# lachinov/brats2019

Hardware: AMD Instinct MI355X
Metric: volumes_per_sec_fwd_bwd_128cubed_x4ch (higher is better)
Workload: dtype bf16

## Files before the change

### brats2019_amd/_lib.py

```python
from __future__ import annotations

import ctypes as C
import os

import torch

_PKG = os.path.dirname(os.path.abspath(__file__))
LIB_PATH = os.environ.get("RU_LIB_PATH") or os.path.join(_PKG, "lib", "libresunet_hip.so")

_lib = None
PRECISIONS = {"f32": 0, "bf16x3": 1}
GRAD_PRECISIONS = {"bf16x3": 1, "bf16": 2}
FUSE_GN_BWD_STATS, FUSE_GN_BWD_APPLY, FUSE_SIDE_STREAM, FUSE_BATCH_WREDUCE, FUSE_TAIL_FINALIZE, FUSE_PW_DGRAD = 1, 2, 4, 8, 16, 32

_vp, _f, _d, _i, _sz = C.c_void_p, C.c_float, C.c_double, C.c_int, C.c_size_t

SIGNATURES = {
    "ru_last_error": (C.c_char_p, []),
    "ru_version": (_i, []),
    "ru_device_ok": (_i, []),
    "ru_conv3d_workspace_bytes": (_sz, [_i] * 7),
    "ru_conv3d_fwd": (_i, [_vp, _vp, _vp, _vp] + [_i] * 7 + [_vp, _sz, _vp]),
    "ru_conv3d_bwd_data": (_i, [_vp, _vp, _vp] + [_i] * 7 + [_vp, _sz, _vp]),
    "ru_conv3d_fwd_p": (_i, [_vp, _vp, _vp, _vp] + [_i] * 8 + [_vp, _sz, _vp]),
# ... 86 lines not shown
    "ru_case_stats": (_i, [_vp, _vp, _i, _i, _i, _i, C.POINTER(_i), C.POINTER(_i), _vp, _sz, _vp]),
    "ru_case_prepare": (_i, [_vp, _vp, _vp, _i, _i, _i, _i, C.POINTER(_i), C.POINTER(_i), C.POINTER(_i), C.POINTER(_i), _i, C.c_uint, _vp]),
    "ru_tta_merge_box": (_i, [_vp, _i, C.c_uint, _vp, _vp, _vp, _i, _i, _i, _i, C.POINTER(_i), C.POINTER(_i), _vp]),
    "ru_cc_workspace_bytes": (_sz, [_i, _i, _i]),
    "ru_cc_reject": (_i, [_vp, _i, _i, _i, _d, _vp, _sz, _vp]),
    "ru_paste_labels": (_i, [_vp, _vp, _i, _i, _i, C.POINTER(_i), C.POINTER(_i), _vp]),
    "ru_postprocess_workspace_bytes": (_sz, [_i, _i, _i, _i]),
    "ru_postprocess_regions": (_i, [_vp, _vp, _i, _i, _i, _i, C.POINTER(C.c_longlong), C.POINTER(C.c_ulonglong), C.c_uint, C.c_uint, _i, _vp, _vp, _vp, _vp, _sz, _vp]),
    "ru_ens_accumulate": (_i, [_vp, _i, C.c_uint, _vp, _i, _i, _i, _i, _i, C.POINTER(_i), C.POINTER(_i), _vp]),
    "ru_ens_finalize": (_i, [_vp, _i, _vp, _vp, _vp, _i, _sz, _vp]),
    "ru_ens_accumulate_finalize": (_i, [_vp, _i, C.c_uint, _vp, _i, _i, _vp, _vp, _vp, _i, _i, _i, _i, C.POINTER(_i), C.POINTER(_i), _vp]),
    "ru_ens_argmax": (_i, [_vp, _i, _vp, _i, _sz, _vp]),
    "ru_paste_probs": (_i, [_vp, _vp, _i, _i, _i, _i, C.POINTER(_i), C.POINTER(_i), _vp]),
    "ru_unc_accumulate": (_i, [_vp, _i, C.c_uint, _vp, _vp, _i, _i, _i, _i, _i, C.POINTER(_i), C.POINTER(_i), _vp]),
    "ru_unc_accumulate_finalize": (_i, [_vp, _i, C.c_uint, _vp, _vp, _i, _i, _i, _vp, _vp, _vp, _vp, _i, _i, _i, _i, C.POINTER(_i), C.POINTER(_i), _vp]),
    "ru_unc_finalize": (_i, [_vp, _vp, _i, _i, _i, _vp, _vp, _vp, _vp, _i, _sz, _vp]),
    "ru_unc_histogram": (_i, [_vp, _vp, _vp, _i, _i, _i, _vp, _vp, _vp]),
    "ru_unc_score": (_i, [_vp, C.POINTER(_i), _i, _vp, _vp, _vp]),
    "ru_paste_u8c": (_i, [_vp, _vp, _i, _i, _i, _i, C.POINTER(_i), C.POINTER(_i), _vp]),
    "ru_zscore_workspace_bytes": (_sz, [_i, _sz]),
    "ru_zscore_stats": (_i, [_vp, _vp, _i, _sz, _vp, _sz, _vp]),
    "ru_augment_patch": (_i, [_vp, _vp, _vp, _vp, _i, _i, _i, _i, _vp, _vp, _vp, _i, _vp, _vp, _vp, _vp, _vp]),
    "ru_augment_patch_soft": (_i, [_vp, _vp, _vp, _vp, _vp, _i, _i, _i, _i, _vp, _vp, _vp, _i, _vp, _vp, _vp, _vp, _vp]),
    "ru_augment_patch_affine": (_i, [_vp, _vp, _vp, _vp, _vp, _i, _i, _i, _i, _vp, _vp, _vp, _i, _vp, _vp, _i, _vp, _vp, _vp]),
    "ru_elastic_workspace_bytes": (_sz, [_i, _i, _i]),
    "ru_elastic_noise": (_i, [C.c_ulonglong, _i, _i, _i, _vp, _vp]),
    "ru_elastic_field": (_i, [_vp, _d, _d, _i, _i, _i, _vp, _vp, _sz, _vp]),
    "ru_elastic_warp": (_i, [_vp, _i, _vp, _i, _vp, _i, _i, _i, _i, _vp, _vp, _vp, _vp, _vp]),
    "ru_intensity_workspace_bytes": (_sz, [_i, _i, _i, _i]),
    "ru_intensity_augment": (_i, [_vp, _vp, _i, _i, _i, _i, _vp, _vp, _sz, _vp]),
    "ru_layout_convert": (_i, [_vp, _vp, _i, _i, _sz, _i, _vp]),
    "ru_upsample2x_trilinear_fwd_l": (_i, [_vp, _vp] + [_i] * 5 + [_f, _vp]),
    "ru_upsample2x_trilinear_bwd_l": (_i, [_vp, _vp] + [_i] * 5 + [_vp]),
    "ru_conv3d_fwd_l": (_i, [_vp, _vp, _vp, _vp] + [_i] * 7 + [_vp, _sz, _vp]),
    "ru_conv3d_bwd_weight_l": (_i, [_vp, _vp, _vp] + [_i] * 7 + [_vp, _sz, _vp]),
    "ru_conv1_l_workspace_bytes": (_sz, [_i, _i, _i]),
    "ru_conv1_l": (_i, [_vp, _i, _vp, _i, _vp, _i, _vp, _vp, _i, _vp, _f, _vp, _f, _i, _i, _sz, _i, _i, _i, _i, _vp, _vp, _f, _vp, _sz,
                        C.POINTER(_i), C.POINTER(_i), _vp, _sz, _vp]),
    "ru_conv3_l_workspace_bytes": (_sz, [_i] * 7),
    "ru_conv3_l": (_i, [_vp, _vp, _vp, _vp] + [_i] * 8 + [_vp, _vp, _vp, _f, _vp, _vp, _i, _i, _vp, _vp, _f, _vp, _sz, C.POINTER(_i), C.POINTER(_i), _vp, _sz, _vp]),
    "ru_wgrad1_l_workspace_bytes": (_sz, [_i, _i, _i, _sz]),
    "ru_wgrad3_l_workspace_bytes": (_sz, [_i] * 7),
    "ru_wgrad3_l": (_i, [_vp, _vp, _vp] + [_i] * 8 + [_vp, _vp, _f, _i, _i, _vp, _vp, _vp, _vp, _vp, _f, _vp, C.POINTER(_i), _vp, _sz, _vp]),
    "ru_wgrad1_l": (_i, [_vp, _vp, _i, _vp, _vp, _i, _i, _i, _i, _sz] + [_i] * 6 + [_vp, _i, _vp, _vp, _f, C.POINTER(_i), _vp, _sz, _vp]),
}


CRIT_KINDS = {"Dice_loss_joint": 0, "BCE_Loss": 1, "MSE_Loss": 2, "CE_Loss": 3, "Dice1D": 4, "GDL_joint": 5, "sens_loss_joint": 6,
              "Dice_loss_separate": 7}
CRIT_MOMENTS, CRIT_MAX_TERMS = 7, 8
CRIT_MASK_LOGS, CRIT_MASK_ALL = (1 << 4) | (1 << 5), 0x7F
CRIT_M_D2 = 6

CONF_PROB, CONF_LABEL, OVERLAP_MAX_LABELS = 0, 1, 8
OVERLAP_MODES = {"itk": 0, "wt": 1, "validate": 2}

UNC_MEASURES = {"std": 0, "entropy": 1}
UNC_REGIONS, UNC_LEVELS, UNC_CLASSES = 3, 101, 4

SURFACE_PROB, SURFACE_LABEL, SURFACE_REGIONS, SURFACE_COUNTS = 0, 1, 3, 6
SURFACE_COLUMNS = {"dice": 0, "sensitivity": 1, "specificity": 2, "hd95": 3}

LESION_COUNTS, LESION_TABLE_COLUMNS, LESION_CHUNK = 6, 5, 8
LESION_COLUMNS = {"dice": 0, "hd95": 1}

POSTPROCESS_MASKS, POSTPROCESS_LABELS, POSTPROCESS_REGIONS, POSTPROCESS_STATS = 0, 1, 3, 6
# ... 77 lines not shown
```

### brats2019_amd/csrc/engine.hip

```cpp
#include "ru_common.h"

#include <vector>
#include <math.h>
#include <stdlib.h>
#include <string.h>

#include <string>
#include <vector>

namespace ru {

static thread_local char g_err[512] = "";
void set_error(const char* fmt, ...) {
    va_list ap;
    va_start(ap, fmt);
    vsnprintf(g_err, sizeof(g_err), fmt, ap);
    va_end(ap);
}
int hip_fail(hipError_t e, const char* what) {
    set_error("%s: %s", what, hipGetErrorString(e));
    return RU_EHIP;
}

constexpr float kSlope = 1e-2f;
// ... 1554 lines not shown

extern "C" int ru_tta_merge(const float* probs, int K, unsigned flips, float* mean_out, unsigned char* mask, unsigned long long* counts,
                            int C, int D, int H, int W, ru_stream_t stream) {
    RU_REQUIRE(probs && mask && counts, "ru_tta_merge: null argument");
    return tta_merge_launch(probs, K, flips, mean_out, mask, counts, C, D, H, W, (hipStream_t)stream);
}
extern "C" int ru_compose_labels(const unsigned char* mask, const unsigned long long* counts, unsigned long long et_min, unsigned char* labels,
                                 size_t V, ru_stream_t stream) {
    RU_REQUIRE(mask && counts && labels, "ru_compose_labels: null argument");
    return compose_labels_launch(mask, counts, et_min, labels, V, (hipStream_t)stream);
}

extern "C" int ru_dice_accumulate(const unsigned long long* counts, double* acc, int N, int C, int nacc, ru_stream_t stream) {
    return dice_accumulate_launch(counts, acc, N, C, nacc, (hipStream_t)stream);
}
extern "C" int ru_dice_counts(const float* p, const float* g, unsigned long long* counts, int N, int C, size_t V, ru_stream_t stream) {
    RU_REQUIRE(p && g && counts && N > 0 && C > 0, "ru_dice_counts: bad argument");
    return dice_counts_launch(p, g, counts, N * C, V, (hipStream_t)stream);
}

extern "C" int ru_layout_convert(const float* src, float* dst, int N, int C, size_t V, int to_c16, ru_stream_t stream) {
    RU_REQUIRE(src && dst && N > 0, "ru_layout_convert: bad argument");
    return layout_convert_launch(src, dst, N, C, V, to_c16, (hipStream_t)stream);
}

extern "C" int ru_upsample2x_trilinear_fwd_l(const float* x, float* y, int N, int C, int D, int H, int W, float out_slope, ru_stream_t stream) {
    RU_REQUIRE(x && y && N > 0 && C > 0 && D > 0 && H > 0 && W > 0, "ru_upsample2x_trilinear_fwd_l: bad argument");
    return up2_fwd16_launch(x, y, N, C, D, H, W, out_slope, (hipStream_t)stream);
}
extern "C" int ru_upsample2x_trilinear_bwd_l(const float* dy, float* dx, int N, int C, int D, int H, int W, ru_stream_t stream) {
    RU_REQUIRE(dy && dx && N > 0 && C > 0 && D > 0 && H > 0 && W > 0, "ru_upsample2x_trilinear_bwd_l: bad argument");
    return up2_bwd16_launch(dy, dx, N, C, D, H, W, (hipStream_t)stream);
}
extern "C" int ru_conv3d_fwd_l(const float* x, const float* w, const float* bias, float* y, int N, int Cin, int Cout, int D, int H, int W,
                               int flags, void* ws, size_t ws_bytes, ru_stream_t stream) {
    RU_REQUIRE(x && w && y, "ru_conv3d_fwd_l: null argument");
    const Switches sw = switches_from_env();
    hipStream_t s = (hipStream_t)stream;
    WsCarver C(ws, ws_bytes);
    Conv3Args a{};
    void* wf = C.take(conv3_sb_frag_bytes(Cin, Cout) / 4 + 64);
    RU_WS_OK(C);
    const bool f32 = (flags & 16) != 0;
    a.products = (flags & 32) ? 2 : 0;
    RU_REQUIRE(!f32 || ((flags & 3) != 0 && !(flags & (4 | 8))), "ru_conv3d_fwd_l: the exact-f32 form needs a voxel-major side and takes neither the 4-channel copy nor a split-form input");
    const bool gop = (flags & 64) && !f32 && (flags & 3) == 3 && !(flags & (4 | 8)) && !bias && conv3_mxg_usable(sw, N, Cin, Cout, D, H, W);
    int rc = f32 ? conv3_f32c_pack_weights(w, wf, Cin, Cout, 0, s) : conv3_sb_pack_weights(w, wf, Cin, Cout, 0, s, gop);
    if (rc) return rc;
    a.mode = f32 ? RU_PREC_F32 : RU_PREC_BF16X3; a.wfrag = wf;
    a.in_c16 = flags & 1; a.out_c16 = (flags >> 1) & 1;
    a.in_s16 = (flags >> 3) & 1;
    RU_REQUIRE(!a.in_s16 || a.in_c16, "ru_conv3d_fwd_l: the split form is a voxel-major layout");
    a.x = x; a.bias = bias; a.y = y; a.N = N; a.Cin = Cin; a.Cout = Cout; a.D = D; a.H = H; a.W = W;
    if (gop) {
        const size_t nvox = (size_t)N * D * H * W;
        float* g16 = C.take(nvox * 16);
        RU_WS_OK(C);
        rc = conv3_mxg_split_launch(x, g16, nvox, s);
        if (rc) return rc;
        a.x = g16; a.in_s16 = 1; a.in_g16 = 1; a.products = 0;
    }
    if (flags & 4) {
        RU_REQUIRE(!(flags & 1) && conv3_sb4_usable(N, Cin, Cout, D, H, W), "ru_conv3d_fwd_l: shape does not fit the 4-channel kernel");
        const size_t V = (size_t)D * H * W;
        float* x4 = C.take((size_t)N * 4 * V);
        void* wf4 = C.take(conv3_sb4_frag_bytes(Cout) / 4 + 64);
// ... 209 lines not shown
```

### brats2019_amd/csrc/pointwise_c16.hip

```cpp
#include "pw_helpers.hpp"
#include "fin_tail.hpp"
#include <type_traits>
#include <stdlib.h>

namespace ru {

typedef float f32x4_c16 __attribute__((ext_vector_type(4)));
template <int I, int N, class F> __device__ __forceinline__ void static_for_c1_impl(F&& f) {
    if constexpr (I < N) { f(std::integral_constant<int, I>{}); static_for_c1_impl<I + 1, N>(f); }
}
template <int N, class F> __device__ __forceinline__ void static_for_c1(F&& f) { static_for_c1_impl<0, N>(f); }

static inline dim3 c16_grid(size_t V, int blocks_nc, unsigned cap = 2048) {
    size_t bx = (V * 4 + 255) / 256;
    if (bx > cap) bx = cap;
    if (bx < 1) bx = 1;
    return dim3((unsigned)bx, (unsigned)blocks_nc);
}

template <int RES, bool NT = false>
__global__ __launch_bounds__(256) void gn_apply16_kernel(const float* __restrict__ x, const float* __restrict__ scale, const float* __restrict__ shift,
                                                         const float* __restrict__ res, float* __restrict__ y, int C, size_t V, float slope,
                                                         const float* __restrict__ rscale, const float* __restrict__ rshift, float rslope) {
    const int nb = blockIdx.y, CB = C >> 4;
// ... 79 lines not shown
        }
    }
#pragma unroll
    for (int k = 0; k < 4; ++k) {
#pragma unroll
        for (int o = 4; o < 64; o <<= 1) { s1[k] += __shfl_xor(s1[k], o); s2[k] += __shfl_xor(s2[k], o); }
    }
    if (lane < 4) {
#pragma unroll
        for (int k = 0; k < 4; ++k) { red[wave][lane * 4 + k][0] = s1[k]; red[wave][lane * 4 + k][1] = s2[k]; }
    }
    __syncthreads();
    if (threadIdx.x < 16) {
        const int c = threadIdx.x;
        float* p = partials + (((size_t)n * C + cb * 16 + c) * nblk + blockIdx.x) * 2;
        stat_publish(p, (red[0][c][0] + red[1][c][0]) + (red[2][c][0] + red[3][c][0]), (red[0][c][1] + red[1][c][1]) + (red[2][c][1] + red[3][c][1]));
    }
    fin_tail(fin, partials, red_dyn + 128);
}
int gn_bwd_reduce16_launch(const float* x, const float* dy, const float* scale, const float* shift, const float* mean, const float* rstd,
                           float slope, float* partials, int N, int C, size_t V, int G, hipStream_t s, const FinTail* fin) {
    RU_REQUIRE(C % 16 == 0 && C % G == 0, "gn_bwd_reduce16: bad channel count");
    const int nblk = gn_bwd_tiles16(V);
    FinTail f{};
    if (fin) f = *fin;
    RU_REQUIRE(!f.ticket || (f.kind == 2 && f.nblk == nblk && f.N == N && f.C == C && f.G == G), "gn_bwd_reduce16: tail descriptor does not match the launch");
    const size_t lds = 512 + fin_tail_lds_bytes(f);
    RU_REQUIRE(lds <= 64 * 1024, "gn_bwd_reduce16: batch x channels too large for the in-launch finalize");
    hipLaunchKernelGGL(gn_bwd_reduce16_kernel, dim3(nblk, N * (C / 16)), dim3(256), lds, s, x, dy, scale, shift, mean, rstd, slope, partials, C, V, G, nblk, gn16_chunk(V), f);
    RU_CHECK_LAUNCH("gn_bwd_reduce16_kernel");
    return RU_OK;
}

__global__ __launch_bounds__(256) void gn_bwd_apply16_kernel(const float* __restrict__ x, const float* __restrict__ dy, const float* __restrict__ scale,
                                                             const float* __restrict__ shift, const float* __restrict__ coef, float slope,
                                                             float* __restrict__ dx, int C, size_t V) {
    const int nb = blockIdx.y, CB = C >> 4;
    const int n = nb / CB, cb = nb - n * CB;
    const int q = threadIdx.x & 3;
    const size_t row = (size_t)n * C + cb * 16 + 4 * q;
    float a[4], b[4], cA[4], cB[4], cC[4];
#pragma unroll
    for (int k = 0; k < 4; ++k) {
        a[k] = scale[row + k]; b[k] = shift[row + k];
        cA[k] = coef[(row + k) * 3]; cB[k] = coef[(row + k) * 3 + 1]; cC[k] = coef[(row + k) * 3 + 2];
    }
    const size_t base = (size_t)nb * V * 4, F = V * 4;
    const float4* xp = reinterpret_cast<const float4*>(x) + base;
    const float4* dp = reinterpret_cast<const float4*>(dy) + base;
    float4* op = reinterpret_cast<float4*>(dx) + base;
    for (size_t f = (size_t)blockIdx.x * 256 + threadIdx.x; f < F; f += (size_t)gridDim.x * 256) {
        const float4 t = xp[f], d = dp[f];
        float4 o;
        o.x = cA[0] * ((t.x * a[0] + b[0]) > 0.f ? d.x : d.x * slope) + (cB[0] * t.x + cC[0]);
        o.y = cA[1] * ((t.y * a[1] + b[1]) > 0.f ? d.y : d.y * slope) + (cB[1] * t.y + cC[1]);
        o.z = cA[2] * ((t.z * a[2] + b[2]) > 0.f ? d.z : d.z * slope) + (cB[2] * t.z + cC[2]);
        o.w = cA[3] * ((t.w * a[3] + b[3]) > 0.f ? d.w : d.w * slope) + (cB[3] * t.w + cC[3]);
        op[f] = o;
    }
}
__global__ __launch_bounds__(256) void gn_bwd_apply16_split_kernel(const float* __restrict__ x, const float* __restrict__ dy, const float* __restrict__ scale,
                                                                   const float* __restrict__ shift, const float* __restrict__ coef, float slope,
                                                                   float* __restrict__ dx, int C, size_t V) {
    const int nb = blockIdx.y, CB = C >> 4;
    const int n = nb / CB, cb = nb - n * CB;
    const int hf = threadIdx.x & 1;
    const size_t row = (size_t)n * C + cb * 16 + 8 * hf;
    float a[8], b[8], cA[8], cB[8], cC[8];
#pragma unroll
    for (int k = 0; k < 8; ++k) {
        a[k] = scale[row + k]; b[k] = shift[row + k];
        cA[k] = coef[(row + k) * 3]; cB[k] = coef[(row + k) * 3 + 1]; cC[k] = coef[(row + k) * 3 + 2];
    }
    const size_t base = (size_t)nb * V * 4, F = V * 2;
    const float4* xp = reinterpret_cast<const float4*>(x) + base;
    const float4* dp = reinterpret_cast<const float4*>(dy) + base;
    pw_u32x4* op = reinterpret_cast<pw_u32x4*>(dx) + base;
    for (size_t f = (size_t)blockIdx.x * 256 + threadIdx.x; f < F; f += (size_t)gridDim.x * 256) {
        const size_t v = f >> 1;
        const float4 t0 = xp[v * 4 + 2 * hf], t1 = xp[v * 4 + 2 * hf + 1], d0 = dp[v * 4 + 2 * hf], d1 = dp[v * 4 + 2 * hf + 1];
        const float tx[8] = {t0.x, t0.y, t0.z, t0.w, t1.x, t1.y, t1.z, t1.w}, dd[8] = {d0.x, d0.y, d0.z, d0.w, d1.x, d1.y, d1.z, d1.w};
        float o[8];
#pragma unroll
        for (int k = 0; k < 8; ++k) o[k] = cA[k] * ((tx[k] * a[k] + b[k]) > 0.f ? dd[k] : dd[k] * slope) + (cB[k] * tx[k] + cC[k]);
        pw_u32x4 hi, lo;
        pw_split8(o, hi, lo);
        op[v * 4 + hf] = hi;
        op[v * 4 + 2 + hf] = lo;
    }
}
int gn_bwd_apply16_launch(const float* x, const float* dy, const float* scale, const float* shift, const float* coef, float slope, float* dx,
                          int N, int C, size_t V, int split, hipStream_t s) {
    RU_REQUIRE(C % 16 == 0, "gn_bwd_apply16: C must be a multiple of 16");
    if (split) {
        size_t bx = (V * 2 + 255) / 256;
        if (bx > 2048) bx = 2048;
        hipLaunchKernelGGL(gn_bwd_apply16_split_kernel, dim3((unsigned)bx, (unsigned)(N * (C / 16))), dim3(256), 0, s, x, dy, scale, shift, coef, slope, dx, C, V);
    } else {
        hipLaunchKernelGGL(gn_bwd_apply16_kernel, c16_grid(V, N * (C / 16)), dim3(256), 0, s, x, dy, scale, shift, coef, slope, dx, C, V);
    }
    RU_CHECK_LAUNCH("gn_bwd_apply16_kernel");
    return RU_OK;
}

__global__ __launch_bounds__(256) void up2_fwd16_kernel(const float* __restrict__ x, float* __restrict__ y, int D, int H, int W, float slope) {
    const int Do = 2 * D, Ho = 2 * H, Wo = 2 * W;
    const size_t nb = blockIdx.y;
    const size_t Vi = (size_t)D * H * W, Vo = Vi * 8;
    const float4* xp = reinterpret_cast<const float4*>(x) + nb * Vi * 4;
    float4* yp = reinterpret_cast<float4*>(y) + nb * Vo * 4;
    const bool nt_out = (size_t)gridDim.y * Vo * 16 * sizeof(float) >= ((size_t)128 << 20);
    const size_t total = (size_t)(D + 1) * (H + 1) * Wo * 4;
    for (size_t f = (size_t)blockIdx.x * 256 + threadIdx.x; f < total; f += (size_t)gridDim.x * 256) {
        const int q = (int)(f & 3);
        size_t r = f >> 2;
        const int xo = (int)(r % Wo); r /= Wo;
        const int ky = (int)(r % (H + 1)) - 1;
        const int kz = (int)(r / (H + 1)) - 1;
        int x0, x1; float lx0, lx1;
        up2_src(xo, W, x0, x1, lx0, lx1);
        const int zA = kz < 0 ? 0 : kz, zB = kz + 1 > D - 1 ? D - 1 : kz + 1;
        const int yA = ky < 0 ? 0 : ky, yB = ky + 1 > H - 1 ? H - 1 : ky + 1;
        const size_t rAA = ((size_t)zA * H + yA) * W, rAB = ((size_t)zA * H + yB) * W, rBA = ((size_t)zB * H + yA) * W, rBB = ((size_t)zB * H + yB) * W;
        const float4 a00 = xp[(rAA + x0) * 4 + q], b00 = xp[(rAA + x1) * 4 + q];
        const float4 a01 = xp[(rAB + x0) * 4 + q], b01 = xp[(rAB + x1) * 4 + q];
        const float4 a10 = xp[(rBA + x0) * 4 + q], b10 = xp[(rBA + x1) * 4 + q];
        const float4 a11 = xp[(rBB + x0) * 4 + q], b11 = xp[(rBB + x1) * 4 + q];
        float4 e00, e01, e10, e11;
#define RU_UPX(c) e00.c = lx0 * a00.c + lx1 * b00.c; e01.c = lx0 * a01.c + lx1 * b01.c; e10.c = lx0 * a10.c + lx1 * b10.c; e11.c = lx0 * a11.c + lx1 * b11.c
        RU_UPX(x); RU_UPX(y); RU_UPX(z); RU_UPX(w);
#undef RU_UPX
#pragma unroll
        for (int dz = 0; dz < 2; ++dz) {
// ... 9 lines not shown
                up2_src(yo, H, y0, y1, ly0, ly1);
                float4 o;
#define RU_UP2(c) o.c = lrelu(lz0 * (ly0 * e00.c + ly1 * e01.c) + lz1 * (ly0 * e10.c + ly1 * e11.c), slope)
                RU_UP2(x); RU_UP2(y); RU_UP2(z); RU_UP2(w);
#undef RU_UP2
                if (nt_out) __builtin_nontemporal_store(f32x4_c16{o.x, o.y, o.z, o.w}, reinterpret_cast<f32x4_c16*>(yp + (((size_t)zo * Ho + yo) * Wo + xo) * 4 + q));
                else yp[(((size_t)zo * Ho + yo) * Wo + xo) * 4 + q] = o;
            }
        }
    }
}
int up2_fwd16_launch(const float* x, float* y, int N, int C, int D, int H, int W, float slope, hipStream_t s) {
    RU_REQUIRE(C % 16 == 0, "up2_fwd16: C must be a multiple of 16");
    const size_t total = (size_t)(D + 1) * (H + 1) * (2 * W) * 4;
    size_t bx = (total + 255) / 256;
    if (bx > 16384) bx = 16384;
    hipLaunchKernelGGL(up2_fwd16_kernel, dim3((unsigned)bx, (unsigned)(N * (C / 16))), dim3(256), 0, s, x, y, D, H, W, slope);
    RU_CHECK_LAUNCH("up2_fwd16_kernel");
    return RU_OK;
}

#ifndef RU_UP2B_ZC
#define RU_UP2B_ZC 8
#endif
constexpr int UP2B_ZC = RU_UP2B_ZC;
__global__ __launch_bounds__(256) void up2_bwd16_kernel(const float* __restrict__ dy, float* __restrict__ dx, int D, int H, int W) {
    const int Do = 2 * D, Ho = 2 * H, Wo = 2 * W;
    const size_t nb = blockIdx.y;
    const size_t Vi = (size_t)D * H * W, Vo = Vi * 8;
    const float4* dp = reinterpret_cast<const float4*>(dy) + nb * Vo * 4;
    float4* op = reinterpret_cast<float4*>(dx) + nb * Vi * 4;
    const int nch = (D + UP2B_ZC - 1) / UP2B_ZC;
    const size_t total = (size_t)nch * H * W * 4;
    for (size_t f = (size_t)blockIdx.x * 256 + threadIdx.x; f < total; f += (size_t)gridDim.x * 256) {
        const int q = (int)(f & 3);
        size_t r = f >> 2;
        const int kx = (int)(r % W); r /= W;
        const int ky = (int)(r % H);
        const int k0 = (int)(r / H) * UP2B_ZC;
        const int k1 = k0 + UP2B_ZC < D ? k0 + UP2B_ZC : D;
        float wy[4], wx[4];
        size_t oy[4], ox[4];
#pragma unroll
        for (int t = 0; t < 4; ++t) {
            const int y = 2 * ky - 1 + t, xx = 2 * kx - 1 + t;
            wy[t] = (y >= 0 && y < Ho) ? up2_coef(y, H, ky) : 0.f;
            wx[t] = (xx >= 0 && xx < Wo) ? up2_coef(xx, W, kx) : 0.f;
            oy[t] = (size_t)(y < 0 ? 0 : (y >= Ho ? Ho - 1 : y)) * Wo;
            ox[t] = (size_t)(xx < 0 ? 0 : (xx >= Wo ? Wo - 1 : xx)) * 4 + q;
        }
        float4 accP = make_float4(0.f, 0.f, 0.f, 0.f), accC = accP;
        for (int m = k0; m <= k1; ++m) {
#pragma unroll
            for (int h = 0; h < 2; ++h) {
                const int z = 2 * m - 1 + h;
                const bool in = z >= 0 && z < Do;
                const size_t zrow = (size_t)(z < 0 ? 0 : (z >= Do ? Do - 1 : z)) * Ho * Wo;
                float4 pz = make_float4(0.f, 0.f, 0.f, 0.f);
#pragma unroll
                for (int b = 0; b < 4; ++b) {
                    const float4* row = dp + (zrow + oy[b]) * 4;
                    const float4 p0 = row[ox[0]], p1 = row[ox[1]], p2 = row[ox[2]], p3 = row[ox[3]];
                    pz.x += wy[b] * (wx[0] * p0.x + wx[1] * p1.x + wx[2] * p2.x + wx[3] * p3.x);
                    pz.y += wy[b] * (wx[0] * p0.y + wx[1] * p1.y + wx[2] * p2.y + wx[3] * p3.y);
                    pz.z += wy[b] * (wx[0] * p0.z + wx[1] * p1.z + wx[2] * p2.z + wx[3] * p3.z);
                    pz.w += wy[b] * (wx[0] * p0.w + wx[1] * p1.w + wx[2] * p2.w + wx[3] * p3.w);
                }
// ... 410 lines not shown
```

### brats2019_amd/csrc/wgrad_f32.hip

```cpp
#include "ru_common.h"

namespace ru {

typedef float f32x4 __attribute__((ext_vector_type(4)));

constexpr int pad2mod4(int v) { return v + ((2 - (v & 3)) & 3); }

template <int TZ, int TY, int OT, int CT>
struct W3 {
    static constexpr int HZ = TZ + 2, HY = TY + 2, HX = 18;
    static constexpr int HVOL = HZ * HY * HX, TVOL = TZ * TY * 16;
    static constexpr int DS = pad2mod4(TVOL), CS = pad2mod4(HVOL);
    static constexpr int LDS_FLOATS = OT * 16 * DS + CT * 16 * CS;
};

template <int NSX, int NSD>
struct W3Slots {
    int gx[NSX];
    int lx[NSX];
    long gd[NSD];
    int n;
};

template <int TZ, int TY, int OT, int CT>
// ... 559 lines not shown
        const int pq = e >> 8, r = (e >> 6) & 3, ln = e & 63;
        const float v = (red[((0 * OT * CT + pq) * 4 + r) * 64 + ln] + red[((1 * OT * CT + pq) * 4 + r) * 64 + ln]) +
                        (red[((2 * OT * CT + pq) * 4 + r) * 64 + ln] + red[((3 * OT * CT + pq) * 4 + r) * 64 + ln]);
        const int p = pq / CT, q = pq - p * CT;
        const int c = c0 + q * 16 + (ln & 15), o = o0 + p * 16 + (ln >> 4) * 4 + r;
        if (o < CoP && c < CiP) partials[((size_t)blockIdx.x * CoP + o) * CiP + c] = v;
    }
}

constexpr int W1S_NG = 4;
__global__ __launch_bounds__(256, 2) void wgrad1_s2d_kernel(const Wgrad1Args a, float* __restrict__ partials, int nchunk, int ncgb, int CoP, int CiP) {
    constexpr int OT = 2, CT = 2, NG = W1S_NG;
    extern __shared__ __attribute__((aligned(16))) float smem[];
    float* dys = smem;
    float* xs = smem + OT * 16 * W1_RS;
    const int tid = threadIdx.x, lane = tid & 63;
    const int wave = __builtin_amdgcn_readfirstlane(tid >> 6);
    const int og = blockIdx.y / ncgb, cgb = blockIdx.y % ncgb;
    const int o0 = og * OT * 16, cbase = cgb * NG * CT * 16;
    const size_t V = a.V;
    const int CBf = a.Cin >> 7;
    const int Hf = 2 * a.Hc, Wf = 2 * a.Wc;
    f32x4 acc[NG][OT][CT];
#pragma unroll
    for (int g = 0; g < NG; ++g)
#pragma unroll
        for (int p = 0; p < OT; ++p)
#pragma unroll
            for (int q = 0; q < CT; ++q) acc[g][p][q] = f32x4{0.f, 0.f, 0.f, 0.f};
    const int abase = (lane & 15) * W1_RS + (lane >> 4) + wave * 64;
    const int q4 = tid & 3, r0 = tid >> 2;
    constexpr int NU = 8;
    const long ntot = (long)a.N * nchunk;
    for (long t = blockIdx.x; t < ntot; t += gridDim.x) {
        const int n = (int)(t / nchunk);
        const size_t v0 = (size_t)(t % nchunk) * W1_VC;
        size_t fv[4];
        bool okv[4];
#pragma unroll
        for (int i = 0; i < 4; ++i) {
            const size_t v = v0 + r0 + 64 * i;
            okv[i] = v < V;
            const size_t vv = okv[i] ? v : 0;
            const int xc = (int)(vv % a.Wc);
            const size_t rr = vv / a.Wc;
            const int yc = (int)(rr % a.Hc), zc = (int)(rr / a.Hc);
            fv[i] = ((size_t)(2 * zc) * Hf + 2 * yc) * Wf + 2 * xc;
        }
        float4 dv[NU], xv[NU];
        auto load_x = [&](int g) __attribute__((always_inline)) {
#pragma unroll
            for (int j = 0; j < NU; ++j) {
                const int p = j >> 2, i = j & 3;
                const int kb = ((cbase + g * CT * 16) >> 4) + p, tap = kb / CBf, cbf = kb - tap * CBf;
                const size_t toff = ((size_t)(tap >> 2) * Hf + ((tap >> 1) & 1)) * Wf + (tap & 1);
                const float4 t4 = *reinterpret_cast<const float4*>(a.x + (((size_t)n * CBf + cbf) * (V * 8) + fv[i] + toff) * 16 + 4 * q4);
                xv[j] = okv[i] ? t4 : make_float4(0.f, 0.f, 0.f, 0.f);
            }
        };
        auto store_x = [&]() __attribute__((always_inline)) {
#pragma unroll
            for (int j = 0; j < NU; ++j) {
                float* d = xs + ((j >> 2) * 16 + 4 * q4) * W1_RS + r0 + 64 * (j & 3);
                d[0] = xv[j].x; d[W1_RS] = xv[j].y; d[2 * W1_RS] = xv[j].z; d[3 * W1_RS] = xv[j].w;
            }
        };
#pragma unroll
        for (int j = 0; j < NU; ++j) {
            const int p = j >> 2, i = j & 3;
            const size_t v = okv[i] ? v0 + r0 + 64 * i : 0;
            const float4 t4 = *reinterpret_cast<const float4*>(a.dy + (((size_t)n * (a.Cout >> 4) + (o0 >> 4) + p) * V + v) * 16 + 4 * q4);
            dv[j] = okv[i] ? t4 : make_float4(0.f, 0.f, 0.f, 0.f);
        }
        load_x(0);
        __syncthreads();
#pragma unroll
        for (int j = 0; j < NU; ++j) {
            float* d = dys + ((j >> 2) * 16 + 4 * q4) * W1_RS + r0 + 64 * (j & 3);
            d[0] = dv[j].x; d[W1_RS] = dv[j].y; d[2 * W1_RS] = dv[j].z; d[3 * W1_RS] = dv[j].w;
        }
        store_x();
        __syncthreads();
#pragma unroll
        for (int g = 0; g < NG; ++g) {
            if (g + 1 < NG) load_x(g + 1);
#pragma unroll
            for (int ks = 0; ks < 16; ++ks) {
                float af[OT], bf[CT];
#pragma unroll
                for (int p = 0; p < OT; ++p) af[p] = dys[abase + p * 16 * W1_RS + ks * 4];
#pragma unroll
                for (int q = 0; q < CT; ++q) bf[q] = xs[abase + q * 16 * W1_RS + ks * 4];
#pragma unroll
                for (int p = 0; p < OT; ++p)
#pragma unroll
                    for (int q = 0; q < CT; ++q)
                        acc[g][p][q] = __builtin_amdgcn_mfma_f32_16x16x4f32(af[p], bf[q], acc[g][p][q], 0, 0, 0);
            }
            if (g + 1 < NG) {
                __syncthreads();
                store_x();
                __syncthreads();
            }
        }
    }
    float* red = smem;
#pragma unroll
    for (int g = 0; g < NG; ++g) {
        __syncthreads();
#pragma unroll
        for (int p = 0; p < OT; ++p)
#pragma unroll
            for (int q = 0; q < CT; ++q)
#pragma unroll
                for (int r = 0; r < 4; ++r) red[((wave * OT * CT + p * CT + q) * 4 + r) * 64 + lane] = acc[g][p][q][r];
        __syncthreads();
        for (int e = tid; e < OT * CT * 256; e += 256) {
            const int pq = e >> 8, r = (e >> 6) & 3, ln = e & 63;
// ... 99 lines not shown
```

### brats2019_amd/ops.py

```python
from __future__ import annotations

import collections
import ctypes as C

import torch

from . import _lib as L

LEAKY_SLOPE = 1e-2


def _dims5(x):
    if x.dim() != 5:
        raise ValueError("expected an NCDHW tensor, got shape %s" % (tuple(x.shape),))
    return [int(v) for v in x.shape]


def _prep(t):
    L.require_gpu()
    if t is None:
        return None
    return t.contiguous().float() if (not t.is_contiguous() or t.dtype != torch.float32) else t


# ... 744 lines not shown


def to_c16(x):
    x = _prep(x)
    n, c, d, h, w = _dims5(x)
    y = torch.empty((n, c // 16, d, h, w, 16), dtype=torch.float32, device=x.device)
    L.check(L.load().ru_layout_convert(L.f32(x), L.f32(y), n, c, d * h * w, 1, L.stream()), "ru_layout_convert")
    return y


def from_c16(x):
    x = _prep(x)
    n, cb, d, h, w, _ = (int(v) for v in x.shape)
    y = torch.empty((n, cb * 16, d, h, w), dtype=torch.float32, device=x.device)
    L.check(L.load().ru_layout_convert(L.f32(x), L.f32(y), n, cb * 16, d * h * w, 0, L.stream()), "ru_layout_convert")
    return y


def upsample2x_c16(x, out_slope=1.0):
    x = _prep(x)
    n, cb, d, h, w, _ = (int(v) for v in x.shape)
    y = torch.empty((n, cb, 2 * d, 2 * h, 2 * w, 16), dtype=torch.float32, device=x.device)
    L.check(L.load().ru_upsample2x_trilinear_fwd_l(L.f32(x), L.f32(y), n, cb * 16, d, h, w, float(out_slope), L.stream()),
            "ru_upsample2x_trilinear_fwd_l")
    return y


def upsample2x_bwd_c16(dy):
    dy = _prep(dy)
    n, cb, d2, h2, w2, _ = (int(v) for v in dy.shape)
    dx = torch.empty((n, cb, d2 // 2, h2 // 2, w2 // 2, 16), dtype=torch.float32, device=dy.device)
    L.check(L.load().ru_upsample2x_trilinear_bwd_l(L.f32(dy), L.f32(dx), n, cb * 16, d2 // 2, h2 // 2, w2 // 2, L.stream()),
            "ru_upsample2x_trilinear_bwd_l")
    return dx


def to_split_c16(x_c16):
    hi = x_c16.to(torch.bfloat16)
    lo = (x_c16 - hi.to(torch.float32)).to(torch.bfloat16)
    return torch.cat([hi, lo], dim=-1).contiguous().view(torch.float32)


def conv3d_layout(x, w, bias=None, in_c16=False, out_c16=False, few_channels=False, in_split=False, exact_f32=False, activations=False, gradient=False):
    x, w, bias = _prep(x), _prep(w), _prep(bias)
    if in_c16:
        n, cb, d, h, wd, _ = (int(v) for v in x.shape)
        cin = cb * 16
    else:
        n, cin, d, h, wd = _dims5(x)
    cout = int(w.shape[0])
    y = torch.empty((n, cout // 16, d, h, wd, 16) if out_c16 else (n, cout, d, h, wd), dtype=torch.float32, device=x.device)
    lib = L.load()
    ws = L.workspace(lib.ru_conv3d_workspace_bytes(n, cin, cout, d, h, wd, 3) + (n * d * h * wd * 16 + 65536 if few_channels else 0)
                     + (n * d * h * wd * 64 + 65536 if gradient else 0), x.device)
    L.check(lib.ru_conv3d_fwd_l(L.f32(x), L.f32(w), L.ptr(bias, True), L.f32(y), n, cin, cout, d, h, wd,
                                int(in_c16) | (int(out_c16) << 1) | (int(few_channels) << 2) | (int(in_split) << 3) | (int(exact_f32) << 4) | (int(activations) << 5) | (int(gradient) << 6),
                                L.ptr(ws), ws.numel(), L.stream()), "ru_conv3d_fwd_l")
    return y


def conv3d_bwd_weight_layout(x, dy, x_c16=False, dy_c16=False):
    x, dy = _prep(x), _prep(dy)
    if x_c16:
        n, cb, d, h, wd, _ = (int(v) for v in x.shape)
        cin = cb * 16
    else:
# ... 161 lines not shown
```

### include/resunet_hip.h

```cpp
#ifndef RESUNET_HIP_H_
#define RESUNET_HIP_H_

#include <stddef.h>
#include <stdint.h>

#ifdef __cplusplus
extern "C" {
#endif

#define RU_OK 0
#define RU_EINVAL (-1)
#define RU_ENOMEM (-2)
#define RU_EHIP (-3)
#define RU_ESTATE (-4)

#define RU_PREC_F32 0
#define RU_PREC_BF16X3 1
#define RU_PREC_BF16 2

typedef void* ru_stream_t;
typedef struct ru_unet* ru_unet_t;

const char* ru_last_error(void);
int ru_version(void);
// ... 218 lines not shown
int ru_paste_u8c(const unsigned char* src, unsigned char* full, int C, int D, int H, int W, const int* lo, const int* size, ru_stream_t stream);

int ru_layout_convert(const float* src, float* dst, int N, int C, size_t V, int to_c16, ru_stream_t stream);
int ru_conv3d_fwd_l(const float* x, const float* w, const float* bias, float* y,
                    int N, int Cin, int Cout, int D, int H, int W, int flags,
                    void* ws, size_t ws_bytes, ru_stream_t stream);
int ru_conv3d_bwd_weight_l(const float* x, const float* dy, float* dw,
                           int N, int Cin, int Cout, int D, int H, int W, int flags,
                           void* ws, size_t ws_bytes, ru_stream_t stream);

size_t ru_conv1_l_workspace_bytes(int C0, int Cout, int s2d);
int ru_conv1_l(const float* x0, int C0, const float* x1, int C1, const float* w, int ldw, float* y, float* y1, int Cout0,
               const float* add, float out_slope, const float* mask, float mask_slope, int N, int Cout, size_t V,
               int s2d, int Dc, int Hc, int Wc, const float* bst_y, const float* bst_k, float bst_slope,
               float* stat_partials, size_t stat_floats, int* nblk, int* inst, void* ws, size_t ws_bytes, ru_stream_t stream);
size_t ru_conv3_l_workspace_bytes(int N, int Cin, int Cout, int D, int H, int W, int flags);
int ru_conv3_l(const float* x, const float* w, const float* bias, float* y, int N, int Cin, int Cout, int D, int H, int W, int flags, int weight_mode,
               const float* add, const float* in_scale, const float* in_shift, float in_slope, const float* in_res, float* in_sum_out,
               int sigmoid, int products, const float* bst_y, const float* bst_k, float bst_slope, float* stat_partials, size_t stat_floats,
               int* nblk, int* route, void* ws, size_t ws_bytes, ru_stream_t stream);
size_t ru_wgrad1_l_workspace_bytes(int N, int Cin, int Cout, size_t V);
int ru_wgrad1_l(const float* x, const float* x1, int C0, const float* dy, float* dw, int ldw, int N, int Cin, int Cout, size_t V,
                int c16, int s2d, int Dc, int Hc, int Wc, int tap_split, const float* dg_w, int dg_ldw, float* dg_y0, float* dg_y1,
                float dg_mask_slope, int* inst, void* ws, size_t ws_bytes, ru_stream_t stream);
size_t ru_wgrad3_l_workspace_bytes(int N, int Cin, int Cout, int D, int H, int W, int flags);
int ru_wgrad3_l(const float* x, const float* dy, float* dw, int N, int Cin, int Cout, int D, int H, int W, int flags, int products,
                const float* in_scale, const float* in_shift, float in_slope, int dw_cin, int dw_cout,
                const float* gb_y, const float* gb_d, const float* gb_scale, const float* gb_shift, const float* gb_coef, float gb_slope, float* gb_out,
                int* inst, void* ws, size_t ws_bytes, ru_stream_t stream);

int ru_upsample2x_trilinear_fwd_l(const float* x, float* y, int N, int C, int D, int H, int W, float out_slope, ru_stream_t stream);
int ru_upsample2x_trilinear_bwd_l(const float* dy, float* dx, int N, int C, int D, int H, int W, ru_stream_t stream);

int ru_dice_counts(const float* p, const float* g, unsigned long long* counts, int N, int C, size_t V, ru_stream_t stream);
int ru_dice_accumulate(const unsigned long long* counts, double* acc, int N, int C, int nacc, ru_stream_t stream);

size_t ru_hausdorff_workspace_bytes(int N, int C, int D, int H, int W, int mode);
int ru_hausdorff_sq(const float* p, const float* g, int N, int C, int D, int H, int W, int mode, unsigned long long* out,
                    void* ws, size_t ws_bytes, ru_stream_t stream);
int ru_hausdorff_accumulate(const unsigned long long* sq, double* acc, int N, int K, int nacc, int mode, ru_stream_t stream);

#define RU_CONF_PROB 0
#define RU_CONF_LABEL 1
#define RU_OVERLAP_MAX_LABELS 8
#define RU_OVERLAP_ITK 0
#define RU_OVERLAP_WT 1
#define RU_OVERLAP_VALIDATE 2
int ru_label_confusion(const void* pred, const void* target, int kind, int N, int C, size_t V, unsigned long long* conf,
                       unsigned long long* invalid, ru_stream_t stream);
int ru_overlap_accumulate(const unsigned long long* conf, int N, int L, int mode, int nacc, double* acc, double* out, ru_stream_t stream);
int ru_dice1d_accumulate(const unsigned long long* counts, double* acc, int N, int C, int classes, ru_stream_t stream);
int ru_rmse_accumulate(const double* sums, double* acc, ru_stream_t stream);

#define RU_SURFACE_PROB 0
#define RU_SURFACE_LABEL 1
#define RU_SURFACE_REGIONS 3
#define RU_SURFACE_DICE 0
#define RU_SURFACE_SENS 1
#define RU_SURFACE_SPEC 2
#define RU_SURFACE_HD95 3
#define RU_SURFACE_COUNTS 6
#define RU_SURFACE_C_INVALID 5
size_t ru_surface_workspace_bytes(int kind, int N, int C, int D, int H, int W);
int ru_surface_metrics(const void* pred, const void* target, int kind, int N, int C, int D, int H, int W, double empty_value,
                       double* values, unsigned long long* counts, void* ws, size_t ws_bytes, ru_stream_t stream);
int ru_surface_accumulate(const double* values, double* acc, int N, int K, int nacc, int column, ru_stream_t stream);
// ... 63 lines not shown
```

Before: 272.8.

## Unroll GN backward apply, remap upsample bwd blocks, prefetch next wgrad1 tile

The GroupNorm backward apply kernels now process several float4 units per thread, issuing all loads before any compute to raise memory-level parallelism, and use fewer blocks when the grid is large. The trilinear upsample backward kernel permutes block indices in groups of eight, likely to spread neighbouring blocks across cache or XCD partitions. The 1x1 wgrad kernel prefetches the next tile's dy and x while finishing the current tile. A ctypes/Python entry point for the GN apply kernel is also added for testing. The added register pressure from the unrolling and prefetching could reduce occupancy.

Result: no change. 273.5 (median of 6 runs) (+0.3%).

```diff
diff --git a/brats2019_amd/_lib.py b/brats2019_amd/_lib.py
--- a/brats2019_amd/_lib.py
+++ b/brats2019_amd/_lib.py
@@ -142,6 +142,7 @@
     "ru_layout_convert": (_i, [_vp, _vp, _i, _i, _sz, _i, _vp]),
     "ru_upsample2x_trilinear_fwd_l": (_i, [_vp, _vp] + [_i] * 5 + [_f, _vp]),
     "ru_upsample2x_trilinear_bwd_l": (_i, [_vp, _vp] + [_i] * 5 + [_vp]),
+    "ru_gn_bwd_apply_l": (_i, [_vp] * 5 + [_f, _vp, _i, _i, _sz, _i, _vp]),
     "ru_conv3d_fwd_l": (_i, [_vp, _vp, _vp, _vp] + [_i] * 7 + [_vp, _sz, _vp]),
     "ru_conv3d_bwd_weight_l": (_i, [_vp, _vp, _vp] + [_i] * 7 + [_vp, _sz, _vp]),
     "ru_conv1_l_workspace_bytes": (_sz, [_i, _i, _i]),
diff --git a/brats2019_amd/csrc/engine.hip b/brats2019_amd/csrc/engine.hip
--- a/brats2019_amd/csrc/engine.hip
+++ b/brats2019_amd/csrc/engine.hip
@@ -1610,6 +1610,11 @@
     RU_REQUIRE(dy && dx && N > 0 && C > 0 && D > 0 && H > 0 && W > 0, "ru_upsample2x_trilinear_bwd_l: bad argument");
     return up2_bwd16_launch(dy, dx, N, C, D, H, W, (hipStream_t)stream);
 }
+extern "C" int ru_gn_bwd_apply_l(const float* x, const float* dy, const float* scale, const float* shift, const float* coef, float slope, float* dx,
+                                 int N, int C, size_t V, int split, ru_stream_t stream) {
+    RU_REQUIRE(x && dy && scale && shift && coef && dx && N > 0 && C > 0 && V > 0, "ru_gn_bwd_apply_l: bad argument");
+    return gn_bwd_apply16_launch(x, dy, scale, shift, coef, slope, dx, N, C, V, split ? 1 : 0, (hipStream_t)stream);
+}
 extern "C" int ru_conv3d_fwd_l(const float* x, const float* w, const float* bias, float* y, int N, int Cin, int Cout, int D, int H, int W,
                                int flags, void* ws, size_t ws_bytes, ru_stream_t stream) {
     RU_REQUIRE(x && w && y, "ru_conv3d_fwd_l: null argument");
diff --git a/brats2019_amd/csrc/pointwise_c16.hip b/brats2019_amd/csrc/pointwise_c16.hip
--- a/brats2019_amd/csrc/pointwise_c16.hip
+++ b/brats2019_amd/csrc/pointwise_c16.hip
@@ -135,6 +135,16 @@
     return RU_OK;
 }
 
+#ifndef RU_GBA_UNITS
+#define RU_GBA_UNITS 4
+#endif
+constexpr int GBA_U = RU_GBA_UNITS;
+static_assert(GBA_U == 1 || GBA_U == 2 || GBA_U == 4, "RU_GBA_UNITS: 1, 2 or 4");
+constexpr unsigned GBA_CAP = 2048;
+__device__ __forceinline__ float gn_bwd_apply_elem(float t, float d, float a, float b, float cA, float cB, float cC, float slope) {
+    return cA * ((t * a + b) > 0.f ? d : d * slope) + (cB * t + cC);
+}
+template <int U>
 __global__ __launch_bounds__(256) void gn_bwd_apply16_kernel(const float* __restrict__ x, const float* __restrict__ dy, const float* __restrict__ scale,
                                                              const float* __restrict__ shift, const float* __restrict__ coef, float slope,
                                                              float* __restrict__ dx, int C, size_t V) {
@@ -152,16 +162,28 @@
     const float4* xp = reinterpret_cast<const float4*>(x) + base;
     const float4* dp = reinterpret_cast<const float4*>(dy) + base;
     float4* op = reinterpret_cast<float4*>(dx) + base;
-    for (size_t f = (size_t)blockIdx.x * 256 + threadIdx.x; f < F; f += (size_t)gridDim.x * 256) {
-        const float4 t = xp[f], d = dp[f];
-        float4 o;
-        o.x = cA[0] * ((t.x * a[0] + b[0]) > 0.f ? d.x : d.x * slope) + (cB[0] * t.x + cC[0]);
-        o.y = cA[1] * ((t.y * a[1] + b[1]) > 0.f ? d.y : d.y * slope) + (cB[1] * t.y + cC[1]);
-        o.z = cA[2] * ((t.z * a[2] + b[2]) > 0.f ? d.z : d.z * slope) + (cB[2] * t.z + cC[2]);
-        o.w = cA[3] * ((t.w * a[3] + b[3]) > 0.f ? d.w : d.w * slope) + (cB[3] * t.w + cC[3]);
-        op[f] = o;
-    }
-}
+    for (size_t f0 = (size_t)blockIdx.x * (256 * U) + threadIdx.x; f0 < F; f0 += (size_t)gridDim.x * (256 * U)) {
+        float4 t[U], d[U];
+#pragma unroll
+        for (int u = 0; u < U; ++u) {
+            const size_t f = f0 + (size_t)u * 256;
+            const size_t fc = f < F ? f : f0;
+            t[u] = xp[fc]; d[u] = dp[fc];
+        }
+        __builtin_amdgcn_sched_barrier(0);
+#pragma unroll
+        for (int u = 0; u < U; ++u) {
+            const size_t f = f0 + (size_t)u * 256, fc = f < F ? f : f0;
+            float4 o;
+            o.x = gn_bwd_apply_elem(t[u].x, d[u].x, a[0], b[0], cA[0], cB[0], cC[0], slope);
+            o.y = gn_bwd_apply_elem(t[u].y, d[u].y, a[1], b[1], cA[1], cB[1], cC[1], slope);
+            o.z = gn_bwd_apply_elem(t[u].z, d[u].z, a[2], b[2], cA[2], cB[2], cC[2], slope);
+            o.w = gn_bwd_apply_elem(t[u].w, d[u].w, a[3], b[3], cA[3], cB[3], cC[3], slope);
+            op[fc] = o;
+        }
+    }
+}
+template <int U>
 __global__ __launch_bounds__(256) void gn_bwd_apply16_split_kernel(const float* __restrict__ x, const float* __restrict__ dy, const float* __restrict__ scale,
                                                                    const float* __restrict__ shift, const float* __restrict__ coef, float slope,
                                                                    float* __restrict__ dx, int C, size_t V) {
@@ -179,29 +201,48 @@
     const float4* xp = reinterpret_cast<const float4*>(x) + base;
     const float4* dp = reinterpret_cast<const float4*>(dy) + base;
     pw_u32x4* op = reinterpret_cast<pw_u32x4*>(dx) + base;
-    for (size_t f = (size_t)blockIdx.x * 256 + threadIdx.x; f < F; f += (size_t)gridDim.x * 256) {
-        const size_t v = f >> 1;
-        const float4 t0 = xp[v * 4 + 2 * hf], t1 = xp[v * 4 + 2 * hf + 1], d0 = dp[v * 4 + 2 * hf], d1 = dp[v * 4 + 2 * hf + 1];
-        const float tx[8] = {t0.x, t0.y, t0.z, t0.w, t1.x, t1.y, t1.z, t1.w}, dd[8] = {d0.x, d0.y, d0.z, d0.w, d1.x, d1.y, d1.z, d1.w};
-        float o[8];
-#pragma unroll
-        for (int k = 0; k < 8; ++k) o[k] = cA[k] * ((tx[k] * a[k] + b[k]) > 0.f ? dd[k] : dd[k] * slope) + (cB[k] * tx[k] + cC[k]);
-        pw_u32x4 hi, lo;
-        pw_split8(o, hi, lo);
-        op[v * 4 + hf] = hi;
-        op[v * 4 + 2 + hf] = lo;
-    }
+    for (size_t f0 = (size_t)blockIdx.x * (256 * U) + threadIdx.x; f0 < F; f0 += (size_t)gridDim.x * (256 * U)) {
+        float4 t0[U], t1[U], d0[U], d1[U];
+#pragma unroll
+        for (int u = 0; u < U; ++u) {
+            const size_t f = f0 + (size_t)u * 256;
+            const size_t v = (f < F ? f : f0) >> 1;
+            t0[u] = xp[v * 4 + 2 * hf]; t1[u] = xp[v * 4 + 2 * hf + 1]; d0[u] = dp[v * 4 + 2 * hf]; d1[u] = dp[v * 4 + 2 * hf + 1];
+        }
+        __builtin_amdgcn_sched_barrier(0);
+#pragma unroll
+        for (int u = 0; u < U; ++u) {
+            const size_t f = f0 + (size_t)u * 256, v = (f < F ? f : f0) >> 1;
+            const float tx[8] = {t0[u].x, t0[u].y, t0[u].z, t0[u].w, t1[u].x, t1[u].y, t1[u].z, t1[u].w};
+            const float dd[8] = {d0[u].x, d0[u].y, d0[u].z, d0[u].w, d1[u].x, d1[u].y, d1[u].z, d1[u].w};
+            float o[8];
+#pragma unroll
+            for (int k = 0; k < 8; ++k) o[k] = gn_bwd_apply_elem(tx[k], dd[k], a[k], b[k], cA[k], cB[k], cC[k], slope);
+            pw_u32x4 hi, lo;
+            pw_split8(o, hi, lo);
+            op[v * 4 + hf] = hi;
+            op[v * 4 + 2 + hf] = lo;
+        }
+    }
+}
+static inline int gn_bwd_apply16_units(size_t units, int blocks_nc) {
+    const size_t bx = (units + (size_t)256 * GBA_U - 1) / ((size_t)256 * GBA_U);
+    return bx * (size_t)blocks_nc >= 2048 ? GBA_U : 1;
 }
 int gn_bwd_apply16_launch(const float* x, const float* dy, const float* scale, const float* shift, const float* coef, float slope, float* dx,
                           int N, int C, size_t V, int split, hipStream_t s) {
     RU_REQUIRE(C % 16 == 0, "gn_bwd_apply16: C must be a multiple of 16");
-    if (split) {
-        size_t bx = (V * 2 + 255) / 256;
-        if (bx > 2048) bx = 2048;
-        hipLaunchKernelGGL(gn_bwd_apply16_split_kernel, dim3((unsigned)bx, (unsigned)(N * (C / 16))), dim3(256), 0, s, x, dy, scale, shift, coef, slope, dx, C, V);
-    } else {
-        hipLaunchKernelGGL(gn_bwd_apply16_kernel, c16_grid(V, N * (C / 16)), dim3(256), 0, s, x, dy, scale, shift, coef, slope, dx, C, V);
-    }
+    RU_REQUIRE(V > 0, "gn_bwd_apply16: empty volume");
+    const size_t units = V * (split ? 2 : 4);
+    const int nc = N * (C / 16), u = gn_bwd_apply16_units(split ? units : units / 2, nc), per = 256 * (split || u == 1 ? u : 2 * u);
+    size_t bx = (units + per - 1) / per;
+    if (bx > GBA_CAP / u) bx = GBA_CAP / u;
+    const dim3 grid((unsigned)bx, (unsigned)nc);
+#define RU_GBA_LAUNCH(U_)                                                                                                                  \
+    if (split) hipLaunchKernelGGL(gn_bwd_apply16_split_kernel<U_>, grid, dim3(256), 0, s, x, dy, scale, shift, coef, slope, dx, C, V);     \
+    else hipLaunchKernelGGL(gn_bwd_apply16_kernel<(U_ == 1 ? 1 : 2 * U_)>, grid, dim3(256), 0, s, x, dy, scale, shift, coef, slope, dx, C, V)
+    if (u == GBA_U) { RU_GBA_LAUNCH(GBA_U); } else { RU_GBA_LAUNCH(1); }
+#undef RU_GBA_LAUNCH
     RU_CHECK_LAUNCH("gn_bwd_apply16_kernel");
     return RU_OK;
 }
@@ -277,7 +318,8 @@
     float4* op = reinterpret_cast<float4*>(dx) + nb * Vi * 4;
     const int nch = (D + UP2B_ZC - 1) / UP2B_ZC;
     const size_t total = (size_t)nch * H * W * 4;
-    for (size_t f = (size_t)blockIdx.x * 256 + threadIdx.x; f < total; f += (size_t)gridDim.x * 256) {
+    const unsigned lb = (gridDim.x & 7) == 0 ? (blockIdx.x & 7) * (gridDim.x >> 3) + (blockIdx.x >> 3) : blockIdx.x;
+    for (size_t f = (size_t)lb * 256 + threadIdx.x; f < total; f += (size_t)gridDim.x * 256) {
         const int q = (int)(f & 3);
         size_t r = f >> 2;
         const int kx = (int)(r % W); r /= W;
diff --git a/brats2019_amd/csrc/wgrad_f32.hip b/brats2019_amd/csrc/wgrad_f32.hip
--- a/brats2019_amd/csrc/wgrad_f32.hip
+++ b/brats2019_amd/csrc/wgrad_f32.hip
@@ -615,11 +615,14 @@
     const int q4 = tid & 3, r0 = tid >> 2;
     constexpr int NU = 8;
     const long ntot = (long)a.N * nchunk;
-    for (long t = blockIdx.x; t < ntot; t += gridDim.x) {
-        const int n = (int)(t / nchunk);
-        const size_t v0 = (size_t)(t % nchunk) * W1_VC;
-        size_t fv[4];
-        bool okv[4];
+    int n = 0;
+    size_t v0 = 0;
+    size_t fv[4];
+    bool okv[4];
+    float4 dv[NU], xv[NU];
+    auto locate = [&](long t) __attribute__((always_inline)) {
+        n = (int)(t / nchunk);
+        v0 = (size_t)(t % nchunk) * W1_VC;
 #pragma unroll
         for (int i = 0; i < 4; ++i) {
             const size_t v = v0 + r0 + 64 * i;
@@ -630,24 +633,25 @@
             const int yc = (int)(rr % a.Hc), zc = (int)(rr / a.Hc);
             fv[i] = ((size_t)(2 * zc) * Hf + 2 * yc) * Wf + 2 * xc;
         }
-        float4 dv[NU], xv[NU];
-        auto load_x = [&](int g) __attribute__((always_inline)) {
-#pragma unroll
-            for (int j = 0; j < NU; ++j) {
-                const int p = j >> 2, i = j & 3;
-                const int kb = ((cbase + g * CT * 16) >> 4) + p, tap = kb / CBf, cbf = kb - tap * CBf;
-                const size_t toff = ((size_t)(tap >> 2) * Hf + ((tap >> 1) & 1)) * Wf + (tap & 1);
-                const float4 t4 = *reinterpret_cast<const float4*>(a.x + (((size_t)n * CBf + cbf) * (V * 8) + fv[i] + toff) * 16 + 4 * q4);
-                xv[j] = okv[i] ? t4 : make_float4(0.f, 0.f, 0.f, 0.f);
-            }
-        };
-        auto store_x = [&]() __attribute__((always_inline)) {
-#pragma unroll
-            for (int j = 0; j < NU; ++j) {
-                float* d = xs + ((j >> 2) * 16 + 4 * q4) * W1_RS + r0 + 64 * (j & 3);
-                d[0] = xv[j].x; d[W1_RS] = xv[j].y; d[2 * W1_RS] = xv[j].z; d[3 * W1_RS] = xv[j].w;
-            }
-        };
+    };
+    auto load_x = [&](int g) __attribute__((always_inline)) {
+#pragma unroll
+        for (int j = 0; j < NU; ++j) {
+            const int p = j >> 2, i = j & 3;
+            const int kb = ((cbase + g * CT * 16) >> 4) + p, tap = kb / CBf, cbf = kb - tap * CBf;
+            const size_t toff = ((size_t)(tap >> 2) * Hf + ((tap >> 1) & 1)) * Wf + (tap & 1);
+            const float4 t4 = *reinterpret_cast<const float4*>(a.x + (((size_t)n * CBf + cbf) * (V * 8) + fv[i] + toff) * 16 + 4 * q4);
+            xv[j] = okv[i] ? t4 : make_float4(0.f, 0.f, 0.f, 0.f);
+        }
+    };
+    auto store_x = [&]() __attribute__((always_inline)) {
+#pragma unroll
+        for (int j = 0; j < NU; ++j) {
+            float* d = xs + ((j >> 2) * 16 + 4 * q4) * W1_RS + r0 + 64 * (j & 3);
+            d[0] = xv[j].x; d[W1_RS] = xv[j].y; d[2 * W1_RS] = xv[j].z; d[3 * W1_RS] = xv[j].w;
+        }
+    };
+    auto load_dy = [&]() __attribute__((always_inline)) {
 #pragma unroll
         for (int j = 0; j < NU; ++j) {
             const int p = j >> 2, i = j & 3;
@@ -655,7 +659,9 @@
             const float4 t4 = *reinterpret_cast<const float4*>(a.dy + (((size_t)n * (a.Cout >> 4) + (o0 >> 4) + p) * V + v) * 16 + 4 * q4);
             dv[j] = okv[i] ? t4 : make_float4(0.f, 0.f, 0.f, 0.f);
         }
-        load_x(0);
+    };
+    if ((long)blockIdx.x < ntot) { locate(blockIdx.x); load_dy(); load_x(0); }
+    for (long t = blockIdx.x; t < ntot; t += gridDim.x) {
         __syncthreads();
 #pragma unroll
         for (int j = 0; j < NU; ++j) {
@@ -667,6 +673,7 @@
 #pragma unroll
         for (int g = 0; g < NG; ++g) {
             if (g + 1 < NG) load_x(g + 1);
+            else if (t + gridDim.x < ntot) { locate(t + gridDim.x); load_dy(); load_x(0); }
 #pragma unroll
             for (int ks = 0; ks < 16; ++ks) {
                 float af[OT], bf[CT];
diff --git a/brats2019_amd/ops.py b/brats2019_amd/ops.py
--- a/brats2019_amd/ops.py
+++ b/brats2019_amd/ops.py
@@ -800,6 +800,17 @@
     dx = torch.empty((n, cb, d2 // 2, h2 // 2, w2 // 2, 16), dtype=torch.float32, device=dy.device)
     L.check(L.load().ru_upsample2x_trilinear_bwd_l(L.f32(dy), L.f32(dx), n, cb * 16, d2 // 2, h2 // 2, w2 // 2, L.stream()),
             "ru_upsample2x_trilinear_bwd_l")
+    return dx
+
+
+def gn_bwd_apply_c16(x, dy, scale, shift, coef, slope=LEAKY_SLOPE, split=True):
+    x, dy, scale, shift, coef = _prep(x), _prep(dy), _prep(scale), _prep(shift), _prep(coef)
+    n, cb, d, h, w, _ = (int(v) for v in x.shape)
+    c = cb * 16
+    assert tuple(dy.shape) == tuple(x.shape) and tuple(scale.shape) == (n, c) and tuple(shift.shape) == (n, c) and tuple(coef.shape) == (n, c, 3)
+    dx = torch.empty_like(x)
+    L.check(L.load().ru_gn_bwd_apply_l(L.f32(x), L.f32(dy), L.f32(scale), L.f32(shift), L.f32(coef), float(slope), L.f32(dx), n, c, d * h * w,
+                                       int(bool(split)), L.stream()), "ru_gn_bwd_apply_l")
     return dx
 
 
diff --git a/include/resunet_hip.h b/include/resunet_hip.h
--- a/include/resunet_hip.h
+++ b/include/resunet_hip.h
@@ -274,6 +274,9 @@
 int ru_upsample2x_trilinear_fwd_l(const float* x, float* y, int N, int C, int D, int H, int W, float out_slope, ru_stream_t stream);
 int ru_upsample2x_trilinear_bwd_l(const float* dy, float* dx, int N, int C, int D, int H, int W, ru_stream_t stream);
 
+int ru_gn_bwd_apply_l(const float* x, const float* dy, const float* scale, const float* shift, const float* coef, float slope, float* dx,
+                      int N, int C, size_t V, int split, ru_stream_t stream);
+
 int ru_dice_counts(const float* p, const float* g, unsigned long long* counts, int N, int C, size_t V, ru_stream_t stream);
 int ru_dice_accumulate(const unsigned long long* counts, double* acc, int N, int C, int nacc, ru_stream_t stream);
 
```
